# latk/hbetune.rs

Measured on NVIDIA B200. Metric: gp_fit_lml_evals_per_s, higher is better.
Workload: dtype f64

## Files before the change

### hbetune_rs_b200/csrc/hbegp.cu

```cuda
#include <cuda_runtime.h>

#include <algorithm>
#include <chrono>
#include <cmath>
#include <cstdio>
#include <cstdlib>
#include <cstring>
#include <functional>
#include <limits>
#include <condition_variable>
#include <map>
#include <mutex>
#include <string>
#include <thread>
#include <tuple>
#include <vector>

#include "../../include/hbegp.h"
#include "gemm.cuh"
#include "gemm_tf32.cuh"
#include "kernels.cuh"
#include "node_mma.cuh"
#include "lbfgs.h"
#include "adapter.h"
#include "comm.h"

namespace hbegp {

static thread_local std::string g_last_error;

static int fail(int code, const std::string& msg) {
    g_last_error = msg;
    return code;
}

// ... 231 lines not shown
    if (std::fabs(nu - 0.5) <= eps) *nu2 = 1;
    else if (std::fabs(nu - 1.5) <= eps) *nu2 = 3;
    else if (std::fabs(nu - 2.5) <= eps) *nu2 = 5;
    else return fail(HBEGP_ERR_UNSUPPORTED, "Matern kernel with arbitrary values for nu (matern_kernel.rs:79)");
    return HBEGP_OK;
}

template <typename T>
struct ModelT;

template <typename T>
struct Engine : EngineBase {
    DevBuf dX, dY;
    int cap = 0;
    DevBuf A, W, xsT, prm, u, alpha, ldp, tpart, gpart, d_lml, d_grad, d_status;
    struct CachedGraph {
        cudaGraphExec_t exec = nullptr;
        long long kernels = 0;
        unsigned epoch = 0;
    };
    unsigned graph_epoch = 0;
    std::map<std::tuple<int, int, int, int, int>, CachedGraph> graphs;
    bool use_graphs = true;
    bool pad_batches = true;
    bool streams_forced = false;
    T* h_prm = nullptr;
    double* h_out = nullptr;
    int* h_status = nullptr;
    size_t h_prm_bytes = 0, h_out_bytes = 0, h_status_bytes = 0;

// ... 12 lines not shown
        if (!(use_graphs && pad_batches && np <= 2048 && cnt > 4)) return cnt;
        const int padded = std::min(cap, (cnt + 3) / 4 * 4);
        if (padded == cnt) return cnt;
        if (std::find(exact_sizes.begin(), exact_sizes.end(), cnt) != exact_sizes.end()) return cnt;
        if (cnt == pad_last_cnt) pad_repeat++;
        else { pad_last_cnt = cnt; pad_repeat = 1; }
        if (pad_repeat >= 4) {
            exact_sizes.push_back(cnt);
            return cnt;
        }
        return padded;
    }

    ~Engine() override {
        drop_graphs();
        for (DevBuf* b : {&dX, &dY, &A, &W, &xsT, &prm, &u, &alpha, &ldp, &tpart, &gpart, &d_lml, &d_grad, &d_status})
            b->release();
        if (h_prm) cudaFreeHost(h_prm);
        if (h_out) cudaFreeHost(h_out);
        if (h_status) cudaFreeHost(h_status);
    }

    void* dev_x() override { return dX.p; }
    void* dev_y() override { return dY.p; }
    size_t elem_size() const override { return sizeof(T); }
    int alloc_data(long n_, int d_) override { return set_data(n_, d_, nullptr, nullptr, true); }
    const double* dev_lml() const override { return (const double*)d_lml.p; }
    const double* dev_grad() const override { return (const double*)d_grad.p; }
    const int* dev_status() const override { return (const int*)d_status.p; }
    Model* new_empty_model(int nu2, const std::vector<double>& prm_h, double noise_clamped) override;

// ... 37 lines not shown

    size_t per_slot_bytes() const {
        size_t s = 2 * (size_t)np * np * sizeof(T);
        s += (size_t)d * np * sizeof(T) + (size_t)p() * sizeof(T) + 2 * (size_t)np * sizeof(T);
        s += (size_t)(np / TILE) * sizeof(T) + (size_t)nchunks() * np * sizeof(T);
        s += (size_t)ntiles_lower() * p() * sizeof(double) + (size_t)(p() + 1) * sizeof(double) + sizeof(int);
        return s;
    }

    int ensure_capacity(int want) {
        if (n <= 0) return fail(HBEGP_ERR_INVALID, "no training data: call hbegp_set_data first");
        if (want <= cap) return HBEGP_OK;
        size_t limit = ws_limit;
        size_t fr = 0, tot = 0;
        CUDA_TRY(cudaMemGetInfo(&fr, &tot));
        const size_t held = A.bytes + W.bytes + gpart.bytes + tpart.bytes + xsT.bytes;
        if (limit == 0) limit = (size_t)((double)(fr + held + model_pool.held) * 0.7);
        size_t per = per_slot_bytes();
        int fit = (int)std::min<size_t>(limit / per, 4096);
        if (fit < 1) return fail(HBEGP_ERR_NOMEM, "workspace limit too small for one n x n evaluation");
        int newcap = std::min(want, fit);
        if (newcap <= cap) return HBEGP_OK;
        if ((size_t)newcap * per > fr + held) model_pool.clear();
        drop_graphs();
        int rc;
        size_t c = (size_t)newcap;
        if ((rc = A.ensure(c * np * np * sizeof(T)))) return rc;
        if ((rc = W.ensure(c * np * np * sizeof(T)))) return rc;
        if ((rc = xsT.ensure(c * d * np * sizeof(T)))) return rc;
        if ((rc = prm.ensure(c * p() * sizeof(T)))) return rc;
        if ((rc = u.ensure(c * np * sizeof(T)))) return rc;
        if ((rc = alpha.ensure(c * np * sizeof(T)))) return rc;
        if ((rc = ldp.ensure(c * (np / TILE) * sizeof(T)))) return rc;
        if ((rc = tpart.ensure(c * nchunks() * np * sizeof(T)))) return rc;
        if ((rc = gpart.ensure(c * ntiles_lower() * p() * sizeof(double)))) return rc;
        if ((rc = d_lml.ensure(c * sizeof(double)))) return rc;
        if ((rc = d_grad.ensure(c * p() * sizeof(double)))) return rc;
        if ((rc = d_status.ensure(((size_t)c + 1) * sizeof(int)))) return rc;
        if (h_prm_bytes < c * p() * sizeof(T)) {
            if (h_prm) cudaFreeHost(h_prm);
            h_prm_bytes = c * p() * sizeof(T);
            CUDA_TRY(cudaMallocHost((void**)&h_prm, h_prm_bytes));
        }
        if (h_out_bytes < c * (p() + 1) * sizeof(double)) {
            if (h_out) cudaFreeHost(h_out);
            h_out_bytes = c * (p() + 1) * sizeof(double);
            CUDA_TRY(cudaMallocHost((void**)&h_out, h_out_bytes));
        }
        if (h_status_bytes < c * sizeof(int)) {
            if (h_status) cudaFreeHost(h_status);
            h_status_bytes = c * sizeof(int);
            CUDA_TRY(cudaMallocHost((void**)&h_status, h_status_bytes));
        }
// ... 3 lines not shown

    void fill_params(const double* theta, const double* lo, const double* hi, T* out) const {
        out[0] = (T)std::exp(theta[0]);
        for (int k = 1; k < p(); k++) {
            double v = std::exp(theta[k]);
            if (lo && v < lo[k]) v = lo[k];
            else if (hi && hi[k] < v) v = hi[k];
            out[k] = (T)v;
        }
    }

    struct Side {
        cudaStream_t st = nullptr;
        cudaEvent_t a = nullptr, b = nullptr;
    };

    int chol_inv(cudaStream_t st, int s0, int cnt, int r0, int s, Side sd = Side()) {
        T* Ab = (T*)A.p + (size_t)s0 * mstride();
        T* Wb = (T*)W.p + (size_t)s0 * mstride();
        if (s == TILE) {
            CUDA_TRY(launch_prio(k_leaf<T>, dim3(1, 1, cnt), dim3(256), leaf_smem_bytes<T>(), st, Ab, Wb, mstride(), np, r0,
                                 (T*)ldp.p + (size_t)s0 * (np / TILE), np / TILE, (int*)d_status.p + s0));
            launches++;
            return HBEGP_OK;
        }
        if (s == 2 * TILE && use_node128) {
            if (node_v == 2) {
                CUDA_TRY(launch_prio(k_node128_v2<false, T>, dim3(1, 1, cnt), dim3(256), node128_v2_smem_bytes(), st, Ab, Wb, mstride(), np, r0,
                                     (T*)ldp.p + (size_t)s0 * (np / TILE), np / TILE, (int*)d_status.p + s0, (long long*)nullptr));
                launches++;
// ... 17 lines not shown
        T* Ab = (T*)A.p + (size_t)s0 * mstride();
        T* Wb = (T*)W.p + (size_t)s0 * mstride();
        int rc;
        T* A21 = Ab + (long)(r0 + s1) * np + r0;
        T* W21 = Wb + (long)(r0 + s1) * np + r0;
        T* W11 = Wb + (long)r0 * np + r0;
        T* A22 = Ab + (long)(r0 + s1) * np + r0 + s1;
        T* W22 = Wb + (long)(r0 + s1) * np + r0 + s1;
        GemmArgs<T> g{};
        g.lda = g.ldb = g.ldc = np;
        g.sA = g.sB = g.sC = mstride();
        g.rowsumsq = nullptr;
        g.small_ctas = np <= small_tile_np ? small_tile_ctas : 0;
        g.A = A21; g.B = W11; g.C = W21; g.M = s2; g.N = s1; g.K = s1; g.kmode = K_LE_N; g.lower_only = 0;
        g.alpha = T(1); g.beta = T(0);
        CUDA_TRY((launch_gemm_auto<T, true, true>(g, cnt, st, aligned128(), 0))); launches++;
        cudaStream_t st3 = st;
        if (sd.st) {
            CUDA_TRY(cudaEventRecord(sd.a, st));
            CUDA_TRY(cudaStreamWaitEvent(sd.st, sd.a, 0));
            st3 = sd.st;
        }
        g.A = W21; g.B = W11; g.C = A21; g.M = s2; g.N = s1; g.K = s1; g.kmode = K_GE_N; g.lower_only = 0;
        g.alpha = T(1); g.beta = T(0);
        CUDA_TRY((launch_gemm_auto<T, true, false>(g, cnt, st3, aligned128(), 1))); launches++;
        if (sd.st) CUDA_TRY(cudaEventRecord(sd.b, sd.st));
        g.A = W21; g.B = W21; g.C = A22; g.M = s2; g.N = s2; g.K = s1; g.kmode = K_FULL; g.lower_only = 1;
        g.alpha = T(-1); g.beta = T(1);
        CUDA_TRY((launch_gemm_auto<T, true, true>(g, cnt, st, aligned128(), 2))); launches++;
        if ((rc = chol_inv(st, s0, cnt, r0 + s1, s2, sd))) return rc;
        if (sd.st) CUDA_TRY(cudaStreamWaitEvent(st, sd.b, 0));
        g.A = W22; g.B = A21; g.C = W21; g.M = s2; g.N = s1; g.K = s2; g.kmode = K_LE_M; g.lower_only = 0;
        g.alpha = T(-1); g.beta = T(0);
        CUDA_TRY((launch_gemm_auto<T, true, false>(g, cnt, st, aligned128(), 3))); launches++;
        return HBEGP_OK;
    }

    int lauum(cudaStream_t st, T* Ab, T* Wb, int cnt) {
        GemmArgs<T> g{};
        g.lda = g.ldb = g.ldc = np;
        g.sA = g.sB = g.sC = mstride();
        g.A = Wb; g.B = Wb; g.C = Ab; g.M = np; g.N = np; g.K = np; g.kmode = K_GE_M; g.lower_only = 1;
        g.alpha = T(1); g.beta = T(0);
        g.rowsumsq = nullptr;
        g.small_ctas = (np <= small_tile_np && small_tile_kinv) ? small_tile_ctas : 0;
        CUDA_TRY((launch_gemm_auto<T, false, false>(g, cnt, st, aligned128(), 4))); launches++;
        return HBEGP_OK;
    }

    int phase = 3;

    template <int NU2>
    int pipeline_nu(cudaStream_t st, int s0, int cnt, bool want_grad, bool want_kinv, Side sd) {
        T* Ab = (T*)A.p + (size_t)s0 * mstride();
        T* Wb = (T*)W.p + (size_t)s0 * mstride();
        T* xs = (T*)xsT.p + (size_t)s0 * d * np;
        T* pr = (T*)prm.p + (size_t)s0 * p();
        T* ub = (T*)u.p + (size_t)s0 * np;
        T* al = (T*)alpha.p + (size_t)s0 * np;
        T* tp = (T*)tpart.p + (size_t)s0 * nchunks() * np;
        double* gp = (double*)gpart.p + (size_t)s0 * ntiles_lower() * p();
        const size_t xsm = 2 * (size_t)feat_chunk(d) * TILE * sizeof(T);
        if (phase == 5) return lauum(st, Ab, Wb, cnt);
        k_scale_x<T><<<dim3((np + 255) / 256, d, cnt), 256, 0, st>>>((const T*)dX.p, (int)n, d, np, pr, p(), xs);
        launches++;
        k_assemble<T, NU2><<<dim3(ntiles_lower(), 1, cnt), 256, xsm, st>>>(xs, (int)n, d, np, pr, p(), Ab, mstride(), 0);
        launches++;
        CUDA_TRY(cudaGetLastError());
        if (phase < 1) return HBEGP_OK;
        int rc;
        if ((rc = chol_inv(st, s0, cnt, 0, np, sd))) return rc;
        if (phase < 2) return HBEGP_OK;
        const bool split = alpha_side && sd.st && (want_grad || want_kinv);
        cudaStream_t sa = st;
        if (split) {
            CUDA_TRY(cudaEventRecord(sd.a, st));
            CUDA_TRY(cudaStreamWaitEvent(sd.st, sd.a, 0));
            sa = sd.st;
        }
        k_trmv_lower<T><<<dim3(np / 8, 1, cnt), 256, 0, sa>>>(Wb, mstride(), np, (const T*)dY.p, 0, ub, np);
        launches++;
        k_trmv_lower_t_part<T><<<dim3(np / TILE, nchunks(), cnt), 256, 0, sa>>>(Wb, mstride(), np, ub, np, tp, nchunks());
        launches++;
        CUDA_TRY(launch_prio(k_sum_chunks<T>, dim3((np + 255) / 256, 1, cnt), dim3(256), 0, sa, tp, nchunks(), np, al, (long)np));
        launches++;
        if (split) CUDA_TRY(cudaEventRecord(sd.b, sd.st));
        if (want_grad || want_kinv) {
            if ((rc = lauum(st, Ab, Wb, cnt))) return rc;
        }
        if (split) CUDA_TRY(cudaStreamWaitEvent(st, sd.b, 0));
        if (phase < 3) return HBEGP_OK;
        if (want_grad) {
            const size_t gsm = xsm + 2 * TILE * sizeof(T) + 8 * (size_t)(feat_chunk(d) + 2) * sizeof(double);
            k_grad_contract<T, NU2><<<dim3(ntiles_lower(), 1, cnt), 256, gsm, st>>>(
                Ab, mstride(), (int)n, d, np, xs, al, np, pr, p(), gp, (long)ntiles_lower() * p());
            launches++;
        }
        CUDA_TRY(launch_prio(k_finish<T>, dim3(cnt), dim3(256), 0, st, (const T*)dY.p, al, np, (int)n, np, (T*)ldp.p + (size_t)s0 * (np / TILE),
                             np / TILE, gp, (long)ntiles_lower() * p(), ntiles_lower(), p(), (int*)d_status.p + s0, (double*)d_lml.p + s0,
                             (double*)d_grad.p + (size_t)s0 * p(), want_grad ? 1 : 0));
        launches++;
        return HBEGP_OK;
    }
// ... 284 lines not shown
        auto copy_out = [&](const T* src, void* dst, int mode) -> int {
            k_sym_fill<T><<<fg, 256, 0, stream>>>(src, np, (int)n, (T*)tmp.p, mode);
            CUDA_TRY(cudaMemcpyAsync(dst, tmp.p, (size_t)n * n * sizeof(T), cudaMemcpyDeviceToHost, stream));
            CUDA_TRY(cudaStreamSynchronize(stream));
            return HBEGP_OK;
        };
        k_scale_x<T><<<dim3((np + 255) / 256, d, 1), 256, 0, stream>>>((const T*)dX.p, (int)n, d, np, (T*)prm.p, p(), (T*)xsT.p);
        if (nu2 == 5) k_assemble<T, 5><<<dim3(ntiles_lower(), 1, 1), 256, xsm, stream>>>((T*)xsT.p, (int)n, d, np, (T*)prm.p, p(), (T*)A.p, mstride(), 0);
        else if (nu2 == 3) k_assemble<T, 3><<<dim3(ntiles_lower(), 1, 1), 256, xsm, stream>>>((T*)xsT.p, (int)n, d, np, (T*)prm.p, p(), (T*)A.p, mstride(), 0);
        else k_assemble<T, 1><<<dim3(ntiles_lower(), 1, 1), 256, xsm, stream>>>((T*)xsT.p, (int)n, d, np, (T*)prm.p, p(), (T*)A.p, mstride(), 0);
        CUDA_TRY(cudaGetLastError());
        if (k && (rc = copy_out((T*)A.p, k, 1))) { tmp.release(); return rc; }
        if ((rc = chol_inv(stream, 0, 1, 0, np))) { tmp.release(); return rc; }
        if (w && (rc = copy_out((T*)W.p, w, 1))) { tmp.release(); return rc; }
        if (kinv) {
            if ((rc = lauum(stream, (T*)A.p, (T*)W.p, 1))) { tmp.release(); return rc; }
            if ((rc = copy_out((T*)A.p, kinv, 0))) { tmp.release(); return rc; }
        }
        int hs = 0;
        CUDA_TRY(cudaMemcpyAsync(&hs, d_status.p, sizeof(int), cudaMemcpyDeviceToHost, stream));
        CUDA_TRY(cudaStreamSynchronize(stream));
        if (status) *status = hs ? HBEGP_NOT_PD : HBEGP_OK;
        tmp.release();
        return HBEGP_OK;
    }
};

template <typename T>
struct ModelT : Model {
    int predict_chunk_rows() const {
        size_t budget = (size_t)1 << 30;
// ... 435 lines not shown
    if (ntiles_lower() > tile0) {
        k_assemble<T, NU2><<<dim3(ntiles_lower() - tile0, 1, 1), 256, xsm, st>>>(xs, (int)n, d, np, pr, p(), Ab, mstride(), tile0);
        launches++;
    }
    CUDA_TRY(cudaMemcpy2DAsync(Wb, (size_t)np * sizeof(T), prior->W.p, (size_t)prior->np * sizeof(T), (size_t)r1 * sizeof(T), r1,
                               cudaMemcpyDeviceToDevice, st));
    CUDA_TRY(cudaMemcpyAsync(ldp.p, prior->ldp.p, (size_t)q * sizeof(T), cudaMemcpyDeviceToDevice, st));
    int rc;
    if (np > r1 && (rc = merge_node(st, 0, 1, 0, r1, np - r1, Side()))) return rc;
    k_trmv_lower<T><<<dim3(np / 8, 1, 1), 256, 0, st>>>(Wb, mstride(), np, (const T*)dY.p, 0, (T*)u.p, np);
    launches++;
    k_trmv_lower_t_part<T><<<dim3(np / TILE, nchunks(), 1), 256, 0, st>>>(Wb, mstride(), np, (T*)u.p, np, (T*)tpart.p, nchunks());
    launches++;
    k_sum_chunks<T><<<dim3((np + 255) / 256, 1, 1), 256, 0, st>>>((T*)tpart.p, nchunks(), np, (T*)alpha.p, np);
    launches++;
    if (want_kinv && (rc = lauum(st, Ab, Wb, 1))) return rc;
    k_finish<T><<<1, 256, 0, st>>>((const T*)dY.p, (T*)alpha.p, np, (int)n, np, (T*)ldp.p, np / TILE, (double*)gpart.p,
                                  (long)ntiles_lower() * p(), ntiles_lower(), p(), (int*)d_status.p, (double*)d_lml.p,
                                  (double*)d_grad.p, 0);
    launches++;
    CUDA_TRY(cudaGetLastError());
    CUDA_TRY(cudaMemcpyAsync(h_out, d_lml.p, sizeof(double), cudaMemcpyDeviceToHost, st));
    CUDA_TRY(cudaMemcpyAsync(h_status, d_status.p, sizeof(int), cudaMemcpyDeviceToHost, st));
    CUDA_TRY(cudaStreamSynchronize(st));
    return HBEGP_OK;
}

template <typename T>
int Engine<T>::model_extend(Model* prior_, Model** out, double* lml, void* alpha_out, void* kinv_out, int* appended) {
    if (!prior_ || !out) return fail(HBEGP_ERR_INVALID, "model_extend: bad arguments");
    *out = nullptr;
// ... 52 lines not shown
    HBEGP_CFG(128, 128, wm128<T>(), 32, true, false);
    HBEGP_CFG(128, 128, wm128<T>(), 32, false, false);
    HBEGP_CFG(64, 64, 32, 32, true, true);
    HBEGP_CFG(64, 64, 32, 32, true, false);
    HBEGP_CFG(64, 64, 32, 32, false, false);
    if constexpr (std::is_same<T, double>::value) {
        HBEGP_CFG(32, 32, 16, 16, true, true);
        HBEGP_CFG(32, 32, 16, 16, true, false);
        HBEGP_CFG(32, 32, 16, 16, false, false);
    } else {
        HBEGP_CFG(32, 32, 32, 16, true, true);
        HBEGP_CFG(32, 32, 32, 16, true, false);
        HBEGP_CFG(32, 32, 32, 16, false, false);
    }
#undef HBEGP_CFG
    if (std::is_same<T, float>::value) {
        CUDA_TRY((tf32::configure<true, true>()));
        CUDA_TRY((tf32::configure<true, false>()));
        CUDA_TRY((tf32::configure<false, false>()));
    }
    const int big = (int)kMaxFeatureSmem;
    CUDA_TRY(cudaFuncSetAttribute(k_leaf<T, 0>, cudaFuncAttributeMaxDynamicSharedMemorySize, (int)leaf_smem_bytes<T>()));
    CUDA_TRY(cudaFuncSetAttribute(k_node128<T>, cudaFuncAttributeMaxDynamicSharedMemorySize, (int)node128_smem_bytes<T>()));
    CUDA_TRY(cudaFuncSetAttribute(k_node128_v2<false, T>, cudaFuncAttributeMaxDynamicSharedMemorySize, (int)node128_v2_smem_bytes()));
    CUDA_TRY(cudaFuncSetAttribute(k_assemble<T, 1>, cudaFuncAttributeMaxDynamicSharedMemorySize, big));
    CUDA_TRY(cudaFuncSetAttribute(k_assemble<T, 3>, cudaFuncAttributeMaxDynamicSharedMemorySize, big));
    CUDA_TRY(cudaFuncSetAttribute(k_assemble<T, 5>, cudaFuncAttributeMaxDynamicSharedMemorySize, big));
    CUDA_TRY(cudaFuncSetAttribute(k_grad_contract<T, 1>, cudaFuncAttributeMaxDynamicSharedMemorySize, big));
    CUDA_TRY(cudaFuncSetAttribute(k_grad_contract<T, 3>, cudaFuncAttributeMaxDynamicSharedMemorySize, big));
    CUDA_TRY(cudaFuncSetAttribute(k_grad_contract<T, 5>, cudaFuncAttributeMaxDynamicSharedMemorySize, big));
// ... 274 lines not shown
        gemm_tile_pref() = (s64 && atoi(s64) == 128) ? 128 : 64;
        gemm_tile_pref_f32() = (s32 && atoi(s32) == 128) ? 128 : 64;
    }
    {
        const char* t = getenv("HBEGP_TF32");
        const char* tm = getenv("HBEGP_TF32_MIN");
        tf32::enabled() = !(t && atoi(t) == 0);
        tf32::min_extent() = tm ? std::max(64, atoi(tm)) : 256;
        if (const char* cm = getenv("HBEGP_TF32_MASK")) tf32::class_mask() = atoi(cm);
        else tf32::class_mask() = 0x3f;
        if (dtype == HBEGP_F32 && tf32::enabled() && !tf32::encode_fn()) {
            delete e;
            return fail(HBEGP_ERR_CUDA, "ctx_create: cuTensorMapEncodeTiled is not available from this driver (set HBEGP_TF32=0)");
        }
    }
    bool graphs_on = true;
    if (const char* s = getenv("HBEGP_GRAPHS")) graphs_on = atoi(s) != 0;
    if (dtype == HBEGP_F64) { static_cast<Engine<double>*>(e)->streams_forced = forced; static_cast<Engine<double>*>(e)->use_graphs = graphs_on; }
    else { static_cast<Engine<float>*>(e)->streams_forced = forced; static_cast<Engine<float>*>(e)->use_graphs = graphs_on; }
    for (int i = 0; i < nsub; i++) {
        cudaStream_t s;
        cudaEvent_t ev;
        if (cudaStreamCreateWithFlags(&s, cudaStreamNonBlocking) != cudaSuccess ||
            cudaEventCreateWithFlags(&ev, cudaEventDisableTiming) != cudaSuccess) {
            delete e;
            return fail(HBEGP_ERR_CUDA, "ctx_create: could not create streams");
        }
        e->sub.push_back(s);
        e->sub_done.push_back(ev);
        cudaStream_t s2;
// ... 809 lines not shown
```

Before: 445.8.

## Emulate f64 GEMM with int8 tensor-core CRT (Ozaki-style) on tcgen05

Adds an f64 GEMM path that scales rows to integers, splits them into int8 residues modulo up to 16 small moduli, multiplies them with tcgen05 int8 MMAs through TMEM, and rebuilds the f64 result by Chinese-remainder reconstruction. By default it is enabled for one GEMM class (mask 0x10) at extents of 512 and above, with the f64 gemm and lauum calls routed through a new dispatcher. The aim is to swap slow native FP64 throughput on B200 for int8 tensor-core throughput. The cost is extra passes for exponents and residues, extra workspace, and a risk of accuracy loss on adversarially scaled inputs.

```diff
diff --git a/hbetune_rs_b200/csrc/gemm_f64emu.cuh b/hbetune_rs_b200/csrc/gemm_f64emu.cuh
--- /dev/null
+++ b/hbetune_rs_b200/csrc/gemm_f64emu.cuh
@@ -0,0 +1,574 @@
+#pragma once
+#include <cuda.h>
+#include <cuda_runtime.h>
+#include <math.h>
+#include <stdint.h>
+
+#include <climits>
+#include <vector>
+
+#include "gemm_tf32.cuh"
+
+namespace hbegp {
+namespace f64emu {
+
+constexpr int MAXMOD = 16, MINMOD = 8;
+__host__ __device__ constexpr int modulus(int i) {
+    constexpr int t[MAXMOD] = {256, 255, 253, 251, 247, 241, 239, 233, 229, 227, 223, 217, 211, 199, 197, 193};
+    return t[i];
+}
+
+constexpr int BM = 128, BN = 64, BK = 128;
+constexpr int A_TILE = BM * BK, B_TILE = BN * BK, STAGE_BYTES = A_TILE + B_TILE;
+constexpr int STAGES = 6;
+constexpr int NBUF = 4;
+constexpr int TMEM_COLS = NBUF * BN;
+constexpr int THREADS = 320;
+constexpr size_t SMEM_BYTES = (size_t)STAGES * STAGE_BYTES + 1024  + 256 ;
+constexpr int EXP_NAN = INT_MIN;
+
+struct Crt {
+    int nmod;
+    int bits;
+    double invP, P1, P2;
+    double p[MAXMOD], invp[MAXMOD], w1[MAXMOD], w2[MAXMOD];
+};
+
+struct Params {
+    CUtensorMap mapA, mapB;
+    const int* expA;
+    const int* expB;
+    long sExpA, sExpB;
+    double* C;
+    long ldc, sC;
+    int M, N, K;
+    int kmode, lower_only;
+    double alpha, beta;
+    Crt crt;
+};
+
+namespace bigint {
+using Big = std::vector<uint32_t>;
+inline void trim(Big& a) {
+    while (!a.empty() && a.back() == 0) a.pop_back();
+}
+inline Big mul_small(const Big& a, uint32_t m) {
+    Big r;
+    uint64_t c = 0;
+    for (uint32_t x : a) {
+        c += (uint64_t)x * m;
+        r.push_back((uint32_t)c);
+        c >>= 32;
+    }
+    if (c) r.push_back((uint32_t)c);
+    trim(r);
+    return r;
+}
+inline Big div_small(const Big& a, uint32_t m, uint32_t* rem) {
+    Big r(a.size());
+    uint64_t c = 0;
+    for (size_t i = a.size(); i-- > 0;) {
+        c = (c << 32) | a[i];
+        r[i] = (uint32_t)(c / m);
+        c %= m;
+    }
+    trim(r);
+    if (rem) *rem = (uint32_t)c;
+    return r;
+}
+inline int bitlen(const Big& a) {
+    if (a.empty()) return 0;
+    return 32 * (int)(a.size() - 1) + (32 - __builtin_clz(a.back()));
+}
+inline bool bit(const Big& a, int i) { return (size_t)(i >> 5) < a.size() && ((a[i >> 5] >> (i & 31)) & 1u); }
+inline double bits_value(const Big& a, int lo, int hi) {
+    double v = 0.0;
+    for (int i = hi - 1; i >= lo; i--) v = v * 2.0 + (bit(a, i) ? 1.0 : 0.0);
+    return ldexp(v, lo);
+}
+inline double low_bits_truncated(const Big& a, int hi, int keep) {
+    int top = -1;
+    for (int i = hi - 1; i >= 0; i--)
+        if (bit(a, i)) { top = i; break; }
+    if (top < 0) return 0.0;
+    const int lo = top + 1 - keep > 0 ? top + 1 - keep : 0;
+    return bits_value(a, lo, top + 1);
+}
+}
+
+inline Crt make_crt(int nmod) {
+    using namespace bigint;
+    Crt c{};
+    c.nmod = nmod;
+    Big P{1};
+    for (int i = 0; i < nmod; i++) P = mul_small(P, (uint32_t)modulus(i));
+    const int L = bitlen(P);
+    c.bits = L - 1 - 2;
+    const int E1 = L - 36;
+    double pd = 0.0;
+    for (size_t i = P.size(); i-- > 0;) pd = pd * 4294967296.0 + (double)P[i];
+    c.invP = 1.0 / pd;
+    c.P1 = bits_value(P, E1, L);
+    c.P2 = low_bits_truncated(P, E1, 41);
+    for (int i = 0; i < nmod; i++) {
+        const uint32_t p = (uint32_t)modulus(i);
+        uint32_t r = 0;
+        const Big Mi = div_small(P, p, nullptr);
+        div_small(Mi, p, &r);
+        uint32_t inv = 1;
+        while ((uint64_t)r * inv % p != 1) inv++;
+        const Big w = mul_small(Mi, inv);
+        c.p[i] = (double)p;
+        c.invp[i] = 1.0 / (double)p;
+        c.w1[i] = bits_value(w, E1, L);
+        c.w2[i] = low_bits_truncated(w, E1, 45);
+    }
+    return c;
+}
+
+inline const Crt& crt_table(int nmod) {
+    static Crt tab[MAXMOD + 1];
+    static bool init = false;
+    if (!init) {
+        for (int m = MINMOD; m <= MAXMOD; m++) tab[m] = make_crt(m);
+        init = true;
+    }
+    return tab[nmod];
+}
+
+inline int ceil_log2(long k) {
+    int c = 0;
+    while ((1L << c) < k) c++;
+    return c;
+}
+
+enum Range : int { R_FULL = 0, R_LE = 1, R_GE = 2 };
+__device__ __forceinline__ void row_range(int range, int r, int K, int& klo, int& khi) {
+    klo = 0;
+    khi = K;
+    if (range == R_LE) khi = min(K, (r / BK + 1) * BK);
+    else if (range == R_GE) klo = (r / BK) * BK;
+}
+
+template <bool KMAJOR>
+__global__ void __launch_bounds__(256) k_emu_scale(const double* __restrict__ X, long ld, long sX, int rows, int K, int range,
+                                                    int bits, int* __restrict__ ex, long sEx) {
+    __shared__ double smax[8][32];
+    __shared__ int sbad[8][32];
+    const int z = blockIdx.z, tid = threadIdx.x, warp = tid >> 5, lane = tid & 31;
+    const double* Xz = X + (long)z * sX;
+    if (KMAJOR) {
+        for (int q = 0; q < 4; q++) {
+            const int r = blockIdx.x * 32 + warp * 4 + q;
+            double m = 0.0;
+            int bad = 0;
+            if (r < rows) {
+                int klo, khi;
+                row_range(range, r, K, klo, khi);
+                for (int k = klo + lane; k < khi; k += 32) {
+                    const double v = Xz[(long)r * ld + k];
+                    bad |= !isfinite(v);
+                    m = fmax(m, fabs(v));
+                }
+            }
+            for (int o = 16; o > 0; o >>= 1) {
+                m = fmax(m, __shfl_xor_sync(0xffffffffu, m, o));
+                bad |= __shfl_xor_sync(0xffffffffu, bad, o);
+            }
+            if (lane == 0) {
+                smax[0][warp * 4 + q] = m;
+                sbad[0][warp * 4 + q] = bad;
+            }
+        }
+        __syncthreads();
+        if (tid < 32) {
+            const int r = blockIdx.x * 32 + tid;
+            if (r < rows) {
+                int e;
+                frexp(smax[0][tid], &e);
+                ex[(long)z * sEx + r] = sbad[0][tid] ? EXP_NAN : (smax[0][tid] == 0.0 ? 0 : bits - e);
+            }
+        }
+    } else {
+        const int r = blockIdx.x * 32 + lane;
+        double m = 0.0;
+        int bad = 0;
+        if (r < rows) {
+            int klo, khi;
+            row_range(range, r, K, klo, khi);
+            for (int k = klo + warp; k < khi; k += 8) {
+                const double v = Xz[(long)k * ld + r];
+                bad |= !isfinite(v);
+                m = fmax(m, fabs(v));
+            }
+        }
+        smax[warp][lane] = m;
+        sbad[warp][lane] = bad;
+        __syncthreads();
+        if (tid < 32 && r < rows) {
+            for (int w = 1; w < 8; w++) {
+                m = fmax(m, smax[w][lane]);
+                bad |= sbad[w][lane];
+            }
+            int e;
+            frexp(m, &e);
+            ex[(long)z * sEx + r] = bad ? EXP_NAN : (m == 0.0 ? 0 : bits - e);
+        }
+    }
+}
+
+template <bool KMAJOR>
+__global__ void __launch_bounds__(256) k_emu_residues(const double* __restrict__ X, long ld, long sX, int rows, int K, int range,
+                                                       const int* __restrict__ ex, long sEx, int nmod, int8_t* __restrict__ R, long sR) {
+    const int z = blockIdx.z, tid = threadIdx.x;
+    const int r = blockIdx.y * 32 + (KMAJOR ? tid / 8 : tid % 32);
+    const int k0 = blockIdx.x * BK + 16 * (KMAJOR ? tid % 8 : tid / 32);
+    if (r >= rows || k0 >= K) return;
+    int klo, khi;
+    row_range(range, r, K, klo, khi);
+    if (k0 < klo || k0 >= khi) return;
+    const int e = ex[(long)z * sEx + r];
+    const double* Xz = X + (long)z * sX;
+    const bool nan = e == EXP_NAN, mul = e >= -1000 && e <= 1000;
+    const double sc = mul ? ldexp(1.0, e) : 1.0;
+    uint32_t lt[16], lm[16], ll[16];
+#pragma unroll
+    for (int j = 0; j < 16; j++) {
+        const double v = KMAJOR ? Xz[(long)r * ld + k0 + j] : Xz[(long)(k0 + j) * ld + r];
+        const long long x = nan ? 0LL : __double2ll_rn(mul ? v * sc : ldexp(v, e));
+        const unsigned long long u = (unsigned long long)(x + (1LL << 56));
+        lt[j] = (uint32_t)(u >> 40);
+        lm[j] = (uint32_t)((u >> 20) & 0xFFFFF);
+        ll[j] = (uint32_t)(u & 0xFFFFF);
+    }
+    int8_t* out = R + (long)z * sR + (long)r * K + k0;
+    const long mstride = (long)rows * K;
+#pragma unroll
+    for (int i = 0; i < MAXMOD; i++) {
+        if (i < nmod) {
+            const uint32_t p = (uint32_t)modulus(i);
+            const uint32_t c20 = (uint32_t)((1ULL << 20) % p), c40 = (uint32_t)((1ULL << 40) % p);
+            const uint32_t unbias = (p - (uint32_t)((1ULL << 56) % p)) % p;
+            const uint32_t half = (p - 1) / 2;
+            uint32_t packed[4];
+#pragma unroll
+            for (int w = 0; w < 4; w++) {
+                uint32_t word = 0;
+#pragma unroll
+                for (int b = 0; b < 4; b++) {
+                    const int j = 4 * w + b;
+                    const uint32_t v = (lt[j] * c40 + lm[j] * c20 + ll[j] + unbias) % p;
+                    const int sv = v > half ? (int)v - (int)p : (int)v;
+                    word |= (uint32_t)(uint8_t)(int8_t)sv << (8 * b);
+                }
+                packed[w] = word;
+            }
+            *reinterpret_cast<uint4*>(out + (long)i * mstride) = make_uint4(packed[0], packed[1], packed[2], packed[3]);
+        }
+    }
+}
+
+constexpr uint32_t IDESC = (2u << 4) | (1u << 7) | (1u << 10) | ((uint32_t)(BN >> 3) << 17) | ((uint32_t)(BM >> 4) << 24);
+
+__device__ __forceinline__ void mma_i8(uint32_t tmem_d, uint64_t adesc, uint64_t bdesc, uint32_t accumulate) {
+    asm volatile(
+        "{\n\t"
+        ".reg .pred p;\n\t"
+        "setp.ne.b32 p, %4, 0;\n\t"
+        "tcgen05.mma.cta_group::1.kind::i8 [%0], %1, %2, %3, p;\n\t"
+        "}\n" ::"r"(tmem_d),
+        "l"(adesc), "l"(bdesc), "r"(IDESC), "r"(accumulate)
+        : "memory");
+}
+
+__device__ __forceinline__ void tma_load_4d(const CUtensorMap* map, uint64_t* bar, void* dst, int c0, int c1, int c2, int c3) {
+    asm volatile(
+        "cp.async.bulk.tensor.4d.shared::cluster.global.mbarrier::complete_tx::bytes [%0], [%1, {%3, %4, %5, %6}], [%2];" ::"r"(
+            tf32::smem_u32(dst)),
+        "l"(reinterpret_cast<uint64_t>(map)), "r"(tf32::smem_u32(bar)), "r"(c0), "r"(c1), "r"(c2), "r"(c3)
+        : "memory");
+}
+
+__device__ __forceinline__ void tile_coords(const Params& p, int t, int tiles_m, int tiles_n, int& mt, int& nt) {
+    if (p.lower_only) {
+        int r = (int)((sqrtf(4.0f * (float)t + 1.0f) - 1.0f) * 0.5f);
+        while ((long)(r + 1) * (r + 2) <= t) ++r;
+        while ((long)r * (r + 1) > t) --r;
+        mt = r;
+        nt = t - r * (r + 1);
+    } else if (p.kmode == K_LE_M) {
+        mt = tiles_m - 1 - t / tiles_n;
+        nt = t % tiles_n;
+    } else if (p.kmode == K_LE_N) {
+        nt = tiles_n - 1 - t / tiles_m;
+        mt = t % tiles_m;
+    } else {
+        nt = t / tiles_m;
+        mt = t % tiles_m;
+    }
+}
+
+__device__ __forceinline__ void tmem_ld16(uint32_t taddr, uint32_t* r) {
+    asm volatile(
+        "tcgen05.ld.sync.aligned.32x32b.x16.b32 {%0, %1, %2, %3, %4, %5, %6, %7, %8, %9, %10, %11, %12, %13, %14, %15}, [%16];"
+        : "=r"(r[0]), "=r"(r[1]), "=r"(r[2]), "=r"(r[3]), "=r"(r[4]), "=r"(r[5]), "=r"(r[6]), "=r"(r[7]), "=r"(r[8]), "=r"(r[9]),
+          "=r"(r[10]), "=r"(r[11]), "=r"(r[12]), "=r"(r[13]), "=r"(r[14]), "=r"(r[15])
+        : "r"(taddr));
+}
+
+__global__ void __launch_bounds__(THREADS, 1) gemm_f64emu_kernel(const __grid_constant__ Params p) {
+    using namespace tf32;
+    extern __shared__ unsigned char smem_raw[];
+    unsigned char* smem = reinterpret_cast<unsigned char*>((reinterpret_cast<uintptr_t>(smem_raw) + 1023) & ~(uintptr_t)1023);
+    uint64_t* bars = reinterpret_cast<uint64_t*>(smem + (size_t)STAGES * STAGE_BYTES);
+    uint64_t* full = bars;
+    uint64_t* empty = bars + STAGES;
+    uint64_t* accf = bars + 2 * STAGES;
+    uint64_t* acce = accf + NBUF;
+    uint32_t* tmem_slot = reinterpret_cast<uint32_t*>(acce + NBUF);
+
+    const int tid = threadIdx.x, warp = tid >> 5, lane = tid & 31;
+    const int tiles_m = (p.M + BM - 1) / BM, tiles_n = p.N / BN;
+    int mt, nt;
+    tile_coords(p, blockIdx.x, tiles_m, tiles_n, mt, nt);
+    const int m0 = mt * BM, n0 = nt * BN, bz = blockIdx.z;
+    int kbeg = 0, kend = p.K;
+    if (p.kmode == K_LE_N) kend = min(p.K, (n0 + BN + BK - 1) / BK * BK);
+    else if (p.kmode == K_GE_N) kbeg = n0 / BK * BK;
+    else if (p.kmode == K_LE_M) kend = min(p.K, m0 + BM);
+    else if (p.kmode == K_GE_M) kbeg = m0;
+    const int nk = (kend > kbeg && n0 < p.N) ? (kend - kbeg + BK - 1) / BK : 0;
+    const int nmod = p.crt.nmod;
+
+    if (warp == 0 && lane == 0) {
+        for (int s = 0; s < STAGES; s++) {
+            mbar_init(&full[s], 1);
+            mbar_init(&empty[s], 1);
+        }
+        for (int b = 0; b < NBUF; b++) {
+            mbar_init(&accf[b], 1);
+            mbar_init(&acce[b], 8);
+        }
+        asm volatile("fence.mbarrier_init.release.cluster;" ::: "memory");
+        asm volatile("prefetch.tensormap [%0];" ::"l"(reinterpret_cast<uint64_t>(&p.mapA)) : "memory");
+        asm volatile("prefetch.tensormap [%0];" ::"l"(reinterpret_cast<uint64_t>(&p.mapB)) : "memory");
+    }
+    if (warp == 1) {
+        asm volatile("tcgen05.alloc.cta_group::1.sync.aligned.shared::cta.b32 [%0], %1;" ::"r"(smem_u32(tmem_slot)), "r"(TMEM_COLS)
+                     : "memory");
+        asm volatile("tcgen05.relinquish_alloc_permit.cta_group::1.sync.aligned;" ::: "memory");
+    }
+    asm volatile("tcgen05.fence::before_thread_sync;" ::: "memory");
+    __syncthreads();
+    asm volatile("tcgen05.fence::after_thread_sync;" ::: "memory");
+    const uint32_t tmem_base = *tmem_slot;
+    const int total = nmod * nk;
+
+    if (warp == 0) {
+        if (lane == 0) {
+            for (int it = 0; it < total; it++) {
+                const int s = it % STAGES, mod = it / nk, kt = it - mod * nk;
+                mbar_wait(&empty[s], ((it / STAGES) & 1) ^ 1);
+                unsigned char* st = smem + (size_t)s * STAGE_BYTES;
+                mbar_expect_tx(&full[s], STAGE_BYTES);
+                const int k0 = kbeg + kt * BK;
+                tma_load_4d(&p.mapA, &full[s], st, k0, m0, mod, bz);
+                tma_load_4d(&p.mapB, &full[s], st + A_TILE, k0, n0, mod, bz);
+            }
+        }
+    } else if (warp == 1) {
+        if (lane == 0) {
+            for (int it = 0; it < total; it++) {
+                const int s = it % STAGES, mod = it / nk, kt = it - mod * nk, buf = mod % NBUF;
+                if (kt == 0) {
+                    mbar_wait(&acce[buf], ((mod / NBUF) & 1) ^ 1);
+                    asm volatile("tcgen05.fence::after_thread_sync;" ::: "memory");
+                }
+                mbar_wait(&full[s], (it / STAGES) & 1);
+                asm volatile("tcgen05.fence::after_thread_sync;" ::: "memory");
+                const uint32_t a = smem_u32(smem + (size_t)s * STAGE_BYTES), b = a + A_TILE;
+#pragma unroll
+                for (int ks = 0; ks < BK / 32; ks++)
+                    mma_i8(tmem_base + buf * BN, make_desc(a + 32 * ks, 16, 1024, 2), make_desc(b + 32 * ks, 16, 1024, 2),
+                           (kt > 0 || ks > 0) ? 1u : 0u);
+                mma_commit(&empty[s]);
+                if (kt == nk - 1) mma_commit(&accf[buf]);
+            }
+        }
+    } else {
+        const int q = warp & 3, half = (warp - 2) >> 2;
+        const int row = m0 + 32 * q + lane, c0 = 32 * half;
+        const uint32_t taddr = tmem_base + ((uint32_t)(32 * q) << 16) + c0;
+        double s1[32], s2[32];
+#pragma unroll
+        for (int j = 0; j < 32; j++) s1[j] = s2[j] = 0.0;
+        for (int mod = 0; mod < (nk > 0 ? nmod : 0); mod++) {
+            const int buf = mod % NBUF;
+            mbar_wait(&accf[buf], (mod / NBUF) & 1);
+            asm volatile("tcgen05.fence::after_thread_sync;" ::: "memory");
+            const double pm = p.crt.p[mod], ipm = p.crt.invp[mod], w1 = p.crt.w1[mod], w2 = p.crt.w2[mod];
+#pragma unroll
+            for (int h = 0; h < 2; h++) {
+                uint32_t v[16];
+                tmem_ld16(taddr + buf * BN + 16 * h, v);
+                asm volatile("tcgen05.wait::ld.sync.aligned;" ::: "memory");
+                if (h == 1) {
+                    asm volatile("tcgen05.fence::before_thread_sync;" ::: "memory");
+                    __syncwarp();
+                    if (lane == 0) mbar_arrive(&acce[buf]);
+                }
+#pragma unroll
+                for (int j = 0; j < 16; j++) {
+                    const double c = (double)(int)v[j];
+                    const double r = fma(-rint(__dmul_rn(c, ipm)), pm, c);
+                    s1[16 * h + j] = fma(r, w1, s1[16 * h + j]);
+                    s2[16 * h + j] = fma(r, w2, s2[16 * h + j]);
+                }
+            }
+        }
+        if (row < p.M && n0 + c0 < p.N) {
+            const int ea = p.expA[(long)bz * p.sExpA + row];
+            double* crow = p.C + (long)bz * p.sC + (long)row * p.ldc + n0 + c0;
+            const int* eb = p.expB + (long)bz * p.sExpB + n0 + c0;
+            const bool use_beta = p.beta != 0.0;
+            const bool store = !p.lower_only || (row / BN) >= (n0 + c0) / BN;
+            if (store) {
+#pragma unroll
+                for (int j = 0; j < 32; j += 2) {
+                    double out[2];
+#pragma unroll
+                    for (int h = 0; h < 2; h++) {
+                        const double qq = rint(__dmul_rn(s1[j + h], p.crt.invP));
+                        const double d1 = fma(-qq, p.crt.P1, s1[j + h]);
+                        const double d2 = __dsub_rn(s2[j + h], __dmul_rn(qq, p.crt.P2));
+                        const int e2 = eb[j + h];
+                        double x = (ea == EXP_NAN || e2 == EXP_NAN) ? __longlong_as_double(0x7ff8000000000000LL)
+                                                                    : ldexp(__dadd_rn(d1, d2), -(ea + e2));
+                        x = __dmul_rn(p.alpha, x);
+                        out[h] = x;
+                    }
+                    double2* ptr = reinterpret_cast<double2*>(crow + j);
+                    if (use_beta) {
+                        const double2 o = *ptr;
+                        out[0] = __dadd_rn(out[0], __dmul_rn(p.beta, o.x));
+                        out[1] = __dadd_rn(out[1], __dmul_rn(p.beta, o.y));
+                    }
+                    *ptr = make_double2(out[0], out[1]);
+                }
+            }
+        }
+        asm volatile("tcgen05.fence::before_thread_sync;" ::: "memory");
+    }
+    __syncthreads();
+    if (warp == 1) {
+        asm volatile("tcgen05.dealloc.cta_group::1.sync.aligned.b32 %0, %1;" ::"r"(tmem_base), "r"(TMEM_COLS) : "memory");
+    }
+}
+
+inline bool& enabled() {
+    static bool on = true;
+    return on;
+}
+inline int& class_mask() {
+    static int v = 0x10;
+    return v;
+}
+inline int& min_extent() {
+    static int v = 512;
+    return v;
+}
+inline int& num_moduli() {
+    static int v = 16;
+    return v;
+}
+
+struct Workspace {
+    int8_t* res = nullptr;
+    long slot_bytes = 0;
+};
+
+inline long slot_bytes(int nmod, long np) { return (long)nmod * np * np + 8 * np + 256; }
+
+inline bool make_map(CUtensorMap* map, const int8_t* base, int rows, int K, int nmod, long batch_stride, int batch, int box_rows) {
+    tf32::EncodeTiledFn enc = tf32::encode_fn();
+    if (!enc) return false;
+    cuuint64_t dims[4] = {(cuuint64_t)K, (cuuint64_t)rows, (cuuint64_t)nmod, (cuuint64_t)batch};
+    cuuint64_t strides[3] = {(cuuint64_t)K, (cuuint64_t)K * rows, (cuuint64_t)(batch > 1 ? batch_stride : (long)K * rows * nmod)};
+    cuuint32_t box[4] = {(cuuint32_t)BK, (cuuint32_t)box_rows, 1, 1};
+    cuuint32_t estr[4] = {1, 1, 1, 1};
+    CUresult r = enc(map, CU_TENSOR_MAP_DATA_TYPE_UINT8, 4, const_cast<int8_t*>(base), dims, strides, box, estr,
+                     CU_TENSOR_MAP_INTERLEAVE_NONE, CU_TENSOR_MAP_SWIZZLE_128B, CU_TENSOR_MAP_L2_PROMOTION_L2_256B,
+                     CU_TENSOR_MAP_FLOAT_OOB_FILL_NONE);
+    return r == CUDA_SUCCESS;
+}
+
+inline cudaError_t configure() {
+    return cudaFuncSetAttribute(gemm_f64emu_kernel, cudaFuncAttributeMaxDynamicSharedMemorySize, (int)SMEM_BYTES);
+}
+
+template <bool KM>
+inline cudaError_t convert(const double* X, long ld, long sX, int rows, int K, int range, int bits, int nmod, int8_t* R, int* ex,
+                           long slot, int batch, cudaStream_t stream) {
+    k_emu_scale<KM><<<dim3((rows + 31) / 32, 1, batch), 256, 0, stream>>>(X, ld, sX, rows, K, range, bits, ex, slot / 4);
+    k_emu_residues<KM><<<dim3((K + BK - 1) / BK, (rows + 31) / 32, batch), 256, 0, stream>>>(X, ld, sX, rows, K, range, ex, slot / 4,
+                                                                                             nmod, R, slot);
+    return cudaGetLastError();
+}
+
+template <bool AK, bool BKM>
+inline cudaError_t launch(const GemmArgs<double>& a, int batch, cudaStream_t stream, const Workspace& ws, int nmod) {
+    if (batch <= 0 || a.M <= 0 || a.N <= 0) return cudaSuccess;
+    if (nmod < MINMOD || nmod > MAXMOD || a.rowsumsq || a.N % BN || a.M % 64 || a.K % 64 || !ws.res) return cudaErrorNotSupported;
+    if (batch > 1 && (a.sA == 0 || a.sB == 0)) return cudaErrorNotSupported;
+    const bool same = a.A == a.B && AK == BKM && a.M == a.N && a.lda == a.ldb && a.sA == a.sB &&
+                      (a.kmode == K_FULL || (a.kmode == K_GE_M && a.lower_only));
+    const long resA = (long)nmod * a.M * a.K, resB = same ? 0 : (long)nmod * a.N * a.K;
+    const long exA = (resA + resB + 255) / 256 * 256, exB = exA + (a.M + 63) / 64 * 64 * 4;
+    if (exB + (long)a.N * 4 > ws.slot_bytes) return cudaErrorNotSupported;
+    const int rangeA = a.kmode == K_LE_M ? R_LE : a.kmode == K_GE_M ? R_GE : R_FULL;
+    const int rangeB = a.kmode == K_LE_N ? R_LE : (a.kmode == K_GE_N || (a.kmode == K_GE_M && a.lower_only)) ? R_GE : R_FULL;
+    const Crt& crt = crt_table(nmod);
+    const int bits = crt.bits - ceil_log2(a.K), abits = std::min(56, bits / 2), bbits = std::min(56, bits - abits);
+    int8_t* RA = ws.res;
+    int8_t* RB = ws.res + resA;
+    int* EA = reinterpret_cast<int*>(ws.res + exA);
+    int* EB = same ? EA : reinterpret_cast<int*>(ws.res + exB);
+    Params p;
+    if (!make_map(&p.mapA, RA, a.M, a.K, nmod, ws.slot_bytes, batch, BM)) return cudaErrorNotSupported;
+    if (!make_map(&p.mapB, same ? RA : RB, a.N, a.K, nmod, ws.slot_bytes, batch, BN)) return cudaErrorNotSupported;
+    cudaError_t e = convert<AK>(a.A, a.lda, a.sA, a.M, a.K, rangeA, abits, nmod, RA, EA, ws.slot_bytes, batch, stream);
+    if (e != cudaSuccess) return e;
+    if (!same) {
+        e = convert<BKM>(a.B, a.ldb, a.sB, a.N, a.K, rangeB, bbits, nmod, RB, EB, ws.slot_bytes, batch, stream);
+        if (e != cudaSuccess) return e;
+    }
+    p.expA = EA; p.expB = EB;
+    p.sExpA = p.sExpB = ws.slot_bytes / 4;
+    p.C = a.C; p.ldc = a.ldc; p.sC = a.sC;
+    p.M = a.M; p.N = a.N; p.K = a.K;
+    p.kmode = a.kmode; p.lower_only = a.lower_only;
+    p.alpha = a.alpha; p.beta = a.beta;
+    p.crt = crt;
+    const long tm = (a.M + BM - 1) / BM, tn = a.N / BN;
+    const long tiles = a.lower_only ? tm * (tm + 1) : tm * tn;
+    return launch_prio(gemm_f64emu_kernel, dim3((unsigned)tiles, 1, (unsigned)batch), dim3(THREADS), SMEM_BYTES, stream, p);
+}
+
+}
+
+inline bool gemm_uses_f64emu(int M, int N, bool aligned128, int cls, const f64emu::Workspace* ws) {
+    return f64emu::enabled() && ws && ws->res && aligned128 && (M < N ? M : N) >= f64emu::min_extent() &&
+           ((f64emu::class_mask() >> cls) & 1);
+}
+
+template <bool AK, bool BKM>
+inline cudaError_t launch_gemm_f64(const GemmArgs<double>& a, int batch, cudaStream_t stream, bool aligned128, int cls,
+                                   const f64emu::Workspace* ws) {
+    if (gemm_uses_f64emu(a.M, a.N, aligned128, cls, ws)) {
+        const cudaError_t e = f64emu::launch<AK, BKM>(a, batch, stream, *ws, f64emu::num_moduli());
+        if (e != cudaErrorNotSupported) return e;
+    }
+    return launch_gemm<double, AK, BKM>(a, batch, stream);
+}
+
+}
diff --git a/hbetune_rs_b200/csrc/hbegp.cu b/hbetune_rs_b200/csrc/hbegp.cu
--- a/hbetune_rs_b200/csrc/hbegp.cu
+++ b/hbetune_rs_b200/csrc/hbegp.cu
@@ -19,6 +19,7 @@
 #include "../../include/hbegp.h"
 #include "gemm.cuh"
 #include "gemm_tf32.cuh"
+#include "gemm_f64emu.cuh"
 #include "kernels.cuh"
 #include "node_mma.cuh"
 #include "lbfgs.h"
@@ -280,6 +281,8 @@
     DevBuf dX, dY;
     int cap = 0;
     DevBuf A, W, xsT, prm, u, alpha, ldp, tpart, gpart, d_lml, d_grad, d_status;
+    DevBuf emu;
+    long emu_slot = 0;
     struct CachedGraph {
         cudaGraphExec_t exec = nullptr;
         long long kernels = 0;
@@ -322,7 +325,7 @@
 
     ~Engine() override {
         drop_graphs();
-        for (DevBuf* b : {&dX, &dY, &A, &W, &xsT, &prm, &u, &alpha, &ldp, &tpart, &gpart, &d_lml, &d_grad, &d_status})
+        for (DevBuf* b : {&dX, &dY, &A, &W, &xsT, &prm, &u, &alpha, &ldp, &tpart, &gpart, &d_lml, &d_grad, &d_status, &emu})
             b->release();
         if (h_prm) cudaFreeHost(h_prm);
         if (h_out) cudaFreeHost(h_out);
@@ -390,11 +393,20 @@
         size_t limit = ws_limit;
         size_t fr = 0, tot = 0;
         CUDA_TRY(cudaMemGetInfo(&fr, &tot));
-        const size_t held = A.bytes + W.bytes + gpart.bytes + tpart.bytes + xsT.bytes;
+        const size_t held = A.bytes + W.bytes + gpart.bytes + tpart.bytes + xsT.bytes + emu.bytes;
         if (limit == 0) limit = (size_t)((double)(fr + held + model_pool.held) * 0.7);
-        size_t per = per_slot_bytes();
+        const bool want_emu = std::is_same<T, double>::value && f64emu::enabled() && tf32::encode_fn();
+        const size_t emu_per = want_emu ? (size_t)f64emu::slot_bytes(f64emu::num_moduli(), np) : 0;
+        size_t per = per_slot_bytes() + emu_per;
         int fit = (int)std::min<size_t>(limit / per, 4096);
+        if (fit < 1 && emu_per) {
+            per -= emu_per;
+            fit = (int)std::min<size_t>(limit / per, 4096);
+            emu.release();
+            emu_slot = 0;
+        }
         if (fit < 1) return fail(HBEGP_ERR_NOMEM, "workspace limit too small for one n x n evaluation");
+        const bool use_emu = emu_per && per > per_slot_bytes();
         int newcap = std::min(want, fit);
         if (newcap <= cap) return HBEGP_OK;
         if ((size_t)newcap * per > fr + held) model_pool.clear();
@@ -413,6 +425,11 @@
         if ((rc = d_lml.ensure(c * sizeof(double)))) return rc;
         if ((rc = d_grad.ensure(c * p() * sizeof(double)))) return rc;
         if ((rc = d_status.ensure(((size_t)c + 1) * sizeof(int)))) return rc;
+        emu_slot = 0;
+        if (use_emu) {
+            if ((rc = emu.ensure(c * emu_per))) return rc;
+            emu_slot = (long)emu_per;
+        }
         if (h_prm_bytes < c * p() * sizeof(T)) {
             if (h_prm) cudaFreeHost(h_prm);
             h_prm_bytes = c * p() * sizeof(T);
@@ -446,6 +463,20 @@
         cudaStream_t st = nullptr;
         cudaEvent_t a = nullptr, b = nullptr;
     };
+
+    template <bool AK, bool BKM>
+    cudaError_t gemm(const GemmArgs<T>& g, int cnt, cudaStream_t st, int cls, int s0) {
+        if constexpr (std::is_same<T, double>::value) {
+            f64emu::Workspace ws;
+            if (emu.p && emu_slot > 0) {
+                ws.res = (int8_t*)emu.p + (size_t)s0 * emu_slot;
+                ws.slot_bytes = emu_slot;
+            }
+            return launch_gemm_f64<AK, BKM>(g, cnt, st, aligned128(), cls, &ws);
+        } else {
+            return launch_gemm_auto<T, AK, BKM>(g, cnt, st, aligned128(), cls);
+        }
+    }
 
     int chol_inv(cudaStream_t st, int s0, int cnt, int r0, int s, Side sd = Side()) {
         T* Ab = (T*)A.p + (size_t)s0 * mstride();
@@ -493,7 +524,7 @@
         g.small_ctas = np <= small_tile_np ? small_tile_ctas : 0;
         g.A = A21; g.B = W11; g.C = W21; g.M = s2; g.N = s1; g.K = s1; g.kmode = K_LE_N; g.lower_only = 0;
         g.alpha = T(1); g.beta = T(0);
-        CUDA_TRY((launch_gemm_auto<T, true, true>(g, cnt, st, aligned128(), 0))); launches++;
+        CUDA_TRY((gemm<true, true>(g, cnt, st, 0, s0))); launches++;
         cudaStream_t st3 = st;
         if (sd.st) {
             CUDA_TRY(cudaEventRecord(sd.a, st));
@@ -502,20 +533,20 @@
         }
         g.A = W21; g.B = W11; g.C = A21; g.M = s2; g.N = s1; g.K = s1; g.kmode = K_GE_N; g.lower_only = 0;
         g.alpha = T(1); g.beta = T(0);
-        CUDA_TRY((launch_gemm_auto<T, true, false>(g, cnt, st3, aligned128(), 1))); launches++;
+        CUDA_TRY((gemm<true, false>(g, cnt, st3, 1, s0))); launches++;
         if (sd.st) CUDA_TRY(cudaEventRecord(sd.b, sd.st));
         g.A = W21; g.B = W21; g.C = A22; g.M = s2; g.N = s2; g.K = s1; g.kmode = K_FULL; g.lower_only = 1;
         g.alpha = T(-1); g.beta = T(1);
-        CUDA_TRY((launch_gemm_auto<T, true, true>(g, cnt, st, aligned128(), 2))); launches++;
+        CUDA_TRY((gemm<true, true>(g, cnt, st, 2, s0))); launches++;
         if ((rc = chol_inv(st, s0, cnt, r0 + s1, s2, sd))) return rc;
         if (sd.st) CUDA_TRY(cudaStreamWaitEvent(st, sd.b, 0));
         g.A = W22; g.B = A21; g.C = W21; g.M = s2; g.N = s1; g.K = s2; g.kmode = K_LE_M; g.lower_only = 0;
         g.alpha = T(-1); g.beta = T(0);
-        CUDA_TRY((launch_gemm_auto<T, true, false>(g, cnt, st, aligned128(), 3))); launches++;
+        CUDA_TRY((gemm<true, false>(g, cnt, st, 3, s0))); launches++;
         return HBEGP_OK;
     }
 
-    int lauum(cudaStream_t st, T* Ab, T* Wb, int cnt) {
+    int lauum(cudaStream_t st, T* Ab, T* Wb, int cnt, int s0) {
         GemmArgs<T> g{};
         g.lda = g.ldb = g.ldc = np;
         g.sA = g.sB = g.sC = mstride();
@@ -523,7 +554,7 @@
         g.alpha = T(1); g.beta = T(0);
         g.rowsumsq = nullptr;
         g.small_ctas = (np <= small_tile_np && small_tile_kinv) ? small_tile_ctas : 0;
-        CUDA_TRY((launch_gemm_auto<T, false, false>(g, cnt, st, aligned128(), 4))); launches++;
+        CUDA_TRY((gemm<false, false>(g, cnt, st, 4, s0))); launches++;
         return HBEGP_OK;
     }
 
@@ -540,7 +571,7 @@
         T* tp = (T*)tpart.p + (size_t)s0 * nchunks() * np;
         double* gp = (double*)gpart.p + (size_t)s0 * ntiles_lower() * p();
         const size_t xsm = 2 * (size_t)feat_chunk(d) * TILE * sizeof(T);
-        if (phase == 5) return lauum(st, Ab, Wb, cnt);
+        if (phase == 5) return lauum(st, Ab, Wb, cnt, s0);
         k_scale_x<T><<<dim3((np + 255) / 256, d, cnt), 256, 0, st>>>((const T*)dX.p, (int)n, d, np, pr, p(), xs);
         launches++;
         k_assemble<T, NU2><<<dim3(ntiles_lower(), 1, cnt), 256, xsm, st>>>(xs, (int)n, d, np, pr, p(), Ab, mstride(), 0);
@@ -565,7 +596,7 @@
         launches++;
         if (split) CUDA_TRY(cudaEventRecord(sd.b, sd.st));
         if (want_grad || want_kinv) {
-            if ((rc = lauum(st, Ab, Wb, cnt))) return rc;
+            if ((rc = lauum(st, Ab, Wb, cnt, s0))) return rc;
         }
         if (split) CUDA_TRY(cudaStreamWaitEvent(st, sd.b, 0));
         if (phase < 3) return HBEGP_OK;
@@ -880,7 +911,7 @@
         if ((rc = chol_inv(stream, 0, 1, 0, np))) { tmp.release(); return rc; }
         if (w && (rc = copy_out((T*)W.p, w, 1))) { tmp.release(); return rc; }
         if (kinv) {
-            if ((rc = lauum(stream, (T*)A.p, (T*)W.p, 1))) { tmp.release(); return rc; }
+            if ((rc = lauum(stream, (T*)A.p, (T*)W.p, 1, 0))) { tmp.release(); return rc; }
             if ((rc = copy_out((T*)A.p, kinv, 0))) { tmp.release(); return rc; }
         }
         int hs = 0;
@@ -1346,7 +1377,7 @@
     launches++;
     k_sum_chunks<T><<<dim3((np + 255) / 256, 1, 1), 256, 0, st>>>((T*)tpart.p, nchunks(), np, (T*)alpha.p, np);
     launches++;
-    if (want_kinv && (rc = lauum(st, Ab, Wb, 1))) return rc;
+    if (want_kinv && (rc = lauum(st, Ab, Wb, 1, 0))) return rc;
     k_finish<T><<<1, 256, 0, st>>>((const T*)dY.p, (T*)alpha.p, np, (int)n, np, (T*)ldp.p, np / TILE, (double*)gpart.p,
                                   (long)ntiles_lower() * p(), ntiles_lower(), p(), (int*)d_status.p, (double*)d_lml.p,
                                   (double*)d_grad.p, 0);
@@ -1429,6 +1460,7 @@
         HBEGP_CFG(32, 32, 32, 16, false, false);
     }
 #undef HBEGP_CFG
+    if (std::is_same<T, double>::value) CUDA_TRY(f64emu::configure());
     if (std::is_same<T, float>::value) {
         CUDA_TRY((tf32::configure<true, true>()));
         CUDA_TRY((tf32::configure<true, false>()));
@@ -1733,6 +1765,16 @@
             return fail(HBEGP_ERR_CUDA, "ctx_create: cuTensorMapEncodeTiled is not available from this driver (set HBEGP_TF32=0)");
         }
     }
+    {
+        const char* t = getenv("HBEGP_F64EMU");
+        f64emu::enabled() = !(t && atoi(t) == 0);
+        const char* tm = getenv("HBEGP_F64EMU_MIN");
+        f64emu::min_extent() = tm ? std::max(64, atoi(tm)) : 512;
+        const char* cm = getenv("HBEGP_F64EMU_MASK");
+        f64emu::class_mask() = cm ? (atoi(cm) & 0x1d) : 0x10;
+        const char* nm = getenv("HBEGP_F64EMU_MODULI");
+        f64emu::num_moduli() = nm ? std::max(f64emu::MINMOD, std::min(f64emu::MAXMOD, atoi(nm))) : 16;
+    }
     bool graphs_on = true;
     if (const char* s = getenv("HBEGP_GRAPHS")) graphs_on = atoi(s) != 0;
     if (dtype == HBEGP_F64) { static_cast<Engine<double>*>(e)->streams_forced = forced; static_cast<Engine<double>*>(e)->use_graphs = graphs_on; }
diff --git a/probes/f64emu_model.py b/probes/f64emu_model.py
--- /dev/null
+++ b/probes/f64emu_model.py
@@ -0,0 +1,140 @@
+import argparse
+import math
+from fractions import Fraction
+
+import numpy as np
+from scipy.linalg import cholesky, solve_triangular
+
+MODULI = [256, 255, 253, 251, 247, 241, 239, 233, 229, 227, 223, 217, 211, 199, 197, 193]
+
+
+def _bits_value(x, lo, hi):
+    return math.ldexp(float((x >> lo) & ((1 << (hi - lo)) - 1)), lo)
+
+
+def _low_truncated(x, hi, keep):
+    v = x & ((1 << hi) - 1)
+    if v == 0:
+        return 0.0
+    top = v.bit_length()
+    lo = max(0, top - keep)
+    return _bits_value(v, lo, top)
+
+
+def crt(nmod):
+    P = math.prod(MODULI[:nmod])
+    L = P.bit_length()
+    E1 = L - 36
+    c = dict(nmod=nmod, bits=L - 3, invP=1.0 / float(P), P1=_bits_value(P, E1, L), P2=_low_truncated(P, E1, 41), p=[], w1=[], w2=[])
+    for p in MODULI[:nmod]:
+        Mi = P // p
+        w = Mi * pow(Mi % p, -1, p)
+        c["p"].append(float(p))
+        c["w1"].append(_bits_value(w, E1, L))
+        c["w2"].append(_low_truncated(w, E1, 45))
+    return c
+
+
+def _exponents(X, nbits):
+    m = np.max(np.abs(X), axis=1)
+    _, e = np.frexp(m)
+    return np.where(m == 0, 0, nbits - e).astype(np.int64)
+
+
+def _residues(Xi, p):
+    r = np.mod(Xi, p)
+    half = (p - 1) // 2
+    return np.where(r > half, r - p, r)
+
+
+def emulated(A, B, nmod):
+    c = crt(nmod)
+    K = A.shape[1]
+    bits = c["bits"] - math.ceil(math.log2(K))
+    abits = min(56, bits // 2)
+    bbits = min(56, bits - abits)
+    ea, eb = _exponents(A, abits), _exponents(B, bbits)
+    Ai = np.rint(np.ldexp(A, ea[:, None])).astype(np.int64)
+    Bi = np.rint(np.ldexp(B, eb[:, None])).astype(np.int64)
+    s1 = np.zeros((A.shape[0], B.shape[0]))
+    s2 = np.zeros_like(s1)
+    for i, p in enumerate(MODULI[:nmod]):
+        ra, rb = _residues(Ai, p), _residues(Bi, p)
+        cd = (ra @ rb.T).astype(np.float64)
+        r = cd - np.rint(cd * (1.0 / p)) * p
+        s1 = s1 + r * c["w1"][i]
+        s2 = s2 + r * c["w2"][i]
+    q = np.rint(s1 * c["invP"])
+    d1 = s1 - q * c["P1"]
+    d2 = s2 - q * c["P2"]
+    return np.ldexp(d1 + d2, -(ea[:, None] + eb[None, :]))
+
+
+def exact_entries(A, B, idx):
+    out = []
+    for i, j in idx:
+        s = sum(Fraction(float(a)) * Fraction(float(b)) for a, b in zip(A[i], B[j]) if a != 0.0 and b != 0.0)
+        out.append(s)
+    return out
+
+
+def matern52(x, ls, c):
+    d = np.sqrt(np.maximum(((x[:, None, :] - x[None, :, :]) / ls) ** 2, 0).sum(-1))
+    s = math.sqrt(5.0) * d
+    return c * (1 + s + s * s / 3) * np.exp(-s)
+
+
+def cases(n, rng):
+    d = 16
+    x = rng.random((n, d))
+    out = []
+    for ls, noise in ((0.5, 1e-2), (2.0, 1e-4), (1.0, 1e-6)):
+        K = matern52(x, np.full(d, ls), 1.3) + noise * np.eye(n)
+        L = cholesky(K, lower=True)
+        W = solve_triangular(L, np.eye(n), lower=True)
+        out.append((f"K^-1 = W^T W, ls={ls} noise={noise:g}", W.T.copy(), W.T.copy()))
+        h = n // 2
+        out.append((f"trailing L21 L21^T, ls={ls} noise={noise:g}", L[h:, :h].copy(), L[h:, :h].copy()))
+    m = n // 2
+    A = rng.standard_normal((m, m)) * np.ldexp(1.0, rng.integers(-20, 1, (m, 1)))
+    B = rng.standard_normal((m, m)) * np.ldexp(1.0, rng.integers(-20, 1, (1, m)))
+    out.append(("adversarial: row / column scales over 2^20", A, B))
+    S = rng.standard_normal((m, m)) * 1e-6
+    S[np.arange(m), rng.integers(0, m, m)] = 1e3
+    out.append(("adversarial: spiky rows", S, S.copy()))
+    return out
+
+
+def main():
+    ap = argparse.ArgumentParser()
+    ap.add_argument("--n", type=int, default=2048)
+    ap.add_argument("--samples", type=int, default=1500)
+    ap.add_argument("--moduli", default="12,13,14,15,16")
+    args = ap.parse_args()
+    rng = np.random.default_rng(0)
+    nmods = [int(v) for v in args.moduli.split(",")]
+    worst_ok = {}
+    for name, A, B in cases(args.n, rng):
+        idx = list(zip(rng.integers(0, A.shape[0], args.samples), rng.integers(0, B.shape[0], args.samples)))
+        ex = exact_entries(A, B, idx)
+        scale = max(abs(float(v)) for v in ex)
+
+        def err(C):
+            return max(abs(float(Fraction(float(C[i, j])) - e)) for (i, j), e in zip(idx, ex)) / scale
+
+        e64 = err(A @ B.T)
+        line = [f"{name}: fp64 {e64:.2e}"]
+        for nm in nmods:
+            e = err(emulated(A, B, nm))
+            line.append(f"N={nm} {e:.2e}")
+            worst_ok.setdefault(nm, True)
+            if e > e64:
+                worst_ok[nm] = False
+        print("  ".join(line), flush=True)
+    ok = [nm for nm in nmods if worst_ok[nm]]
+    print(f"error relative to max |C| over {args.samples} sampled entries per case, exact reference")
+    print("smallest N no worse than fp64 on every case:", min(ok) if ok else None)
+
+
+if __name__ == "__main__":
+    main()
```

After: 453.8 (median of 6 runs). +1.8%, better.
